# RamSaw/PipelineDP

Measured on AMD Instinct MI355X. Metric: records/sec DPEngine.aggregate COUNT+SUM at 1/2/4/8 MI355X; % HBM roofline, higher is better.
Workload: dtype f64; 1 GPU; configs[1]: 1e+09 records / 1e+07 privacy ids / 1e+06 Zipf(1.1) partitions per GPU, COUNT+SUM+PRIVACY_ID_COUNT, private partition selection; records_per_gpu=1000000000, privacy_ids_per_gpu=10000000, partitions=1000000, max_partitions_contributed=8, max_contributions_per_partition=2, noise=laplace, selection=truncated_geometric, parallelism=pid-sharded x1, privacy_id_range_supplied=True

## Files before the change

### pipelinedp_amd/csrc/dpg_api.hip

```cpp
#include <dlfcn.h>
#include <hip/hip_runtime.h>
#include <rccl/rccl.h>

#include <algorithm>
#include <cstddef>
#include <chrono>
#include <cmath>
#include <cstdio>
#include <cstdlib>
#include <cstring>
#include <map>
#include <mutex>
#include <string>
#include <thread>
#include <tuple>
#include <vector>

static hipError_t occ_query(int *blocks, const void *kern, int threads, size_t lds) {
    static std::mutex mu;
    static std::map<std::tuple<int, const void *, int, size_t>, int> cache;
    int dev = 0;
    (void)hipGetDevice(&dev);
    std::lock_guard<std::mutex> g(mu);
    const auto key = std::make_tuple(dev, kern, threads, lds);
// ... 29 lines not shown
#include "dpg_strkey.h"
#include "dpg_owner.h"
#include "dpg_pairx.h"
#include "dpg_partition.h"
#include "dpg_quantile.h"
#include "dpg_records.h"
#include "dpg_rsort.h"
#include "dpg_sample.h"
#include "dpg_select.h"
#include "dpg_shard.h"
#include "dpg_sortb.h"
#include "dpg_sortmw.h"
#include "dpg_team.h"
#include "dpg_utility.h"
#include "dpg_vsum.h"
#include "dpg_wave.h"
#include "dpg_hist_phases.h"

using namespace dpg;

namespace {

constexpr uint32_t kBucketTarget = 256;
constexpr uint32_t kMaxB1 = 11, kMaxB2 = 12, kMaxBR = 11;
constexpr uint32_t kMaxB1W = 12;
constexpr int kIptL1W = 8;
constexpr uint32_t kPinErr = 4096;
constexpr uint32_t kChunkGroup = 32;
constexpr int kRedoLevel2 = -100;
#ifndef DPG_PC_HALF
#define DPG_PC_HALF 0
#endif
#ifndef DPG_IPT_PC
#define DPG_IPT_PC 8
#endif

struct Buf {
    void *p = nullptr;
    size_t bytes = 0;
};

struct Control {
    uint32_t err;
    uint32_t item_cursor;
    uint32_t ntiles[8];
    int64_t n_scalar;
    uint32_t n_chunks;
    uint32_t n_over;
    uint32_t n_over2;
    uint32_t n_mchunks;
    uint32_t heavy_nfb;
    uint32_t pad_;
    uint32_t seg_paths[2];
    unsigned long long over_records;
    unsigned long long over2_records;
    unsigned long long pid_lo, pid_hi;
};

}

struct dpg_ctx {
    int device = 0;
    uint64_t seed = 0;
    int n_cu = 256;
    std::string err;
    std::map<std::string, Buf> bufs;
    std::vector<std::string> stage_names;
    std::vector<hipEvent_t> events;
    int n_events_used = 0;
    hipStream_t last_stream = nullptr;
    uint32_t bucket_target = 0;
    uint32_t bucket_cap = kBCap;
    void *comm = nullptr;
    const uint32_t *last_err = nullptr;
    int rank = 0, nranks = 1;
    char *stage_buf = nullptr;
    size_t stage_cap = 0, stage_head = 0;
    std::map<hipStream_t, hipEvent_t> stage_done;
    uint32_t *pin_tot = nullptr;
    hipEvent_t tot_ev = nullptr;
    uint32_t team_backoff = 0;
    uint32_t team_backoff_next = 64;
};

namespace {

int watchdog_seconds() {
#if defined(DPG_WATCHDOG) || defined(DPG_PHASE_TIMING)
    const char *e = std::getenv("DPG_WATCHDOG_S");
    return e ? std::atoi(e) : 0;
#else
    return 0;
#endif
}

uint32_t *watchdog_buffer(size_t n) {
    static uint32_t *buf = nullptr;
    static size_t cap = 0;
    if (n > cap) {
        if (buf) (void)hipHostFree(buf);
        if (hipHostMalloc((void **)&buf, n * 4, hipHostMallocCoherent) != hipSuccess) return nullptr;
        cap = n;
    }
    std::memset(buf, 0, n * 4);
    return buf;
}
// ... 1051 lines not shown
    WS(rbase, int64_t, "pieces.rbase", (size_t)8 * F);
    WS(cum, uint32_t, "pieces.cum", (size_t)8 * F);
    WS(tot, uint32_t, "pieces.tot", F);
    WS(ptot, uint32_t, "pieces.ptot", F);
    WS(ostart, int64_t, "pieces.ostart", F);
    WS(pdesc, PieceDesc, "pieces.desc", F);
    HIP_TRY(hipMemsetAsync(cum, 0, (size_t)8 * F * 4, s));
    HIP_TRY(hipMemsetAsync(&ctl->ntiles[0], 0, 4, s));
    stage(ctx, s, "partition1:pieces");
    k_region_base<<<(8 * F + 255) / 256, 256, 0, s>>>(rbase, F, C);
    LAUNCH_CHECK();
    k_build_tiles_single<<<(nt + 255) / 256, 256, 0, s>>>(n, sub, 1u, tiles, stb, snt,
                                                         &ctl->ntiles[0], XcdQueues{});
    LAUNCH_CHECK();
    using Src = SrcSoAKey<R, true>;
    constexpr size_t lds = scatter_lds<Src, R, IPT, FMAX, NT>();
    static_assert(lds <= (size_t)160 * 1024 * NT / kScatThreads - 512, "scatter LDS");
    if (F > (uint32_t)FMAX) return fail(ctx, DPG_ERR_HIP, "internal: piece level fan-out too large");
    auto kern = k_scatter<Src, R, IPT, FMAX, false, NT>;
    if (bits <= (uint32_t)agg_bits()) return fail(ctx, DPG_ERR_HIP, "internal: piece level fan-out");
    (void)set_func_attr((const void *)kern, hipFuncAttributeMaxDynamicSharedMemorySize,
                              (int)lds);
    const uint32_t gs = std::min<uint32_t>(nt, (uint32_t)ctx->n_cu * (kScatThreads / NT));
    if (int r = scat_phase_begin(ctx, s)) return r;
    kern<<<gs, NT, lds, s>>>(src, tiles, &ctl->ntiles[0], F, bits, nullptr, rbase, out,
                             XcdQueues{}, nullptr, nullptr, nullptr, 1u, cum, C,
                             (uint32_t)((uint64_t)8 * F * C), &ctl->err);
    LAUNCH_CHECK();
    if (int r = scat_phase_end(ctx, s, "partition1:pieces", gs)) return r;
    k_piece_totals<<<1, 1024, 0, s>>>(cum, rbase, F, tot, ptot, ostart, pdesc);
    LAUNCH_CHECK();
    if (!ctx->tot_ev && hipEventCreateWithFlags(&ctx->tot_ev, hipEventDisableTiming) != hipSuccess)
        return fail(ctx, DPG_ERR_HIP, "hipEventCreate (totals)");
    HIP_TRY(hipMemcpyAsync(host_tot, tot, (size_t)F * 4, hipMemcpyDeviceToHost, s));
    HIP_TRY(hipMemcpyAsync(host_tot + kPinErr, &ctl->err, 4, hipMemcpyDeviceToHost, s));
    HIP_TRY(hipEventRecord(ctx->tot_ev, s));
    *pt = PieceTab{rbase, cum, tot, ptot, ostart, F, pdesc};
    return DPG_OK;
}

template <class R>
int run_team_level2(dpg_ctx *ctx, hipStream_t s, const SrcAoS<R> &src, uint32_t S, uint32_t F2,
                    const int64_t *seg_start, const uint32_t *seg_cnt, R *out, Control *ctl,
                    int64_t **base_out, uint32_t **tot_out, const PieceTab *pt,
                    uint64_t max_bucket) {
    int st = DPG_OK;
    const uint32_t F = kTeamF;
    const size_t words = (size_t)8 * 3 * F + 8 * kTeamArriveStride + 32;
    WS(tw, uint32_t, "team.sync", words);
    WS(base, int64_t, "partition2.base", (size_t)S * F2);
    WS(tot, uint32_t, "partition2.tot", (size_t)S * F2);
    HIP_TRY(hipMemsetAsync(tw, 0, words * 4, s));
    uint32_t *abort_flag = tw + (size_t)8 * 3 * F + 8 * kTeamArriveStride;
    const TeamSync ts{tw, tw + (size_t)8 * 3 * F, abort_flag, &ctl->err};
    if (std::getenv("DPG_DEBUG_TEAM_ABORT")) {
        const uint32_t one = 1;
        UPLOAD(abort_flag, &one, 4);
        k_set_bits<<<1, 1, 0, s>>>(&ctl->err, 8u);
        LAUNCH_CHECK();
    }
    uint32_t sub_cap = (uint32_t)kTeamSub;
    if (const char *e = std::getenv("DPG_DEBUG_TEAM_SUB"))
        sub_cap = std::min<uint32_t>(sub_cap, std::max<uint32_t>(2, (uint32_t)std::atoi(e)) & ~1u);
    const uint32_t T = (uint32_t)ctx->n_cu / 8;
    const bool multi = (max_bucket + 8 + T - 1) / T + 2 > sub_cap;
    const void *k = pt ? (const void *)k_part2_team<R, true> : (const void *)k_part2_team<R, false>;
    (void)set_func_attr(k, hipFuncAttributeMaxDynamicSharedMemorySize, (int)team_lds<R>());
    stage(ctx, s, "partition2:team");
    if (pt)
        k_part2_team<R, true><<<(unsigned)ctx->n_cu, kScatThreads, team_lds<R>(), s>>>(
            src, seg_start, seg_cnt, S, F2, out, base, tot, ts, *pt, sub_cap);
    else
        k_part2_team<R, false><<<(unsigned)ctx->n_cu, kScatThreads, team_lds<R>(), s>>>(
            src, seg_start, seg_cnt, S, F2, out, base, tot, ts, PieceTab{}, sub_cap);
    LAUNCH_CHECK();
    if (multi) {
        stage(ctx, s, "partition2:team_multi");
        HIP_TRY(hipMemsetAsync(tw, 0, ((size_t)8 * 3 * F + 8 * kTeamArriveStride) * 4, s));
        const void *km = pt ? (const void *)k_part2_team<R, true, true>
                            : (const void *)k_part2_team<R, false, true>;
        (void)set_func_attr(km, hipFuncAttributeMaxDynamicSharedMemorySize, (int)team_lds<R>());
        if (pt)
            k_part2_team<R, true, true><<<(unsigned)ctx->n_cu, kScatThreads, team_lds<R>(), s>>>(
                src, seg_start, seg_cnt, S, F2, out, base, tot, ts, *pt, sub_cap);
        else
            k_part2_team<R, false, true><<<(unsigned)ctx->n_cu, kScatThreads, team_lds<R>(), s>>>(
                src, seg_start, seg_cnt, S, F2, out, base, tot, ts, PieceTab{}, sub_cap);
        LAUNCH_CHECK();
    }
    *base_out = base;
    *tot_out = tot;
    return DPG_OK;
}

template <class R>
int pipeline(dpg_ctx *ctx, hipStream_t s, const int64_t *pid, const int64_t *pk,
             const double *value, int64_t n, const dpg_bound_params *p, const dpg_partials *out,
             Control *ctl, const Plan &pl, int64_t pid_min, uint64_t U, uint32_t ib, PaOut *pa) {
    int st = DPG_OK;
    const bool var = (p->metric_mask & (DPG_M_MEAN | DPG_M_VARIANCE)) != 0;
    const Fmt f{ib, pl.pkbits, pl.kbits, pl.b1};
    const HashK H = make_hash(pl.kbits);
    const uint32_t F1 = 1u << pl.b1;
    SrcSoAKey<R> s1{pid, pk, p->public_mask, pl.P, pid_min, U, H, f,
                    low_mask(pl.kbits - pl.b1 + pl.pkbits), pl.kbits - pl.b1, &ctl->err};
    s1.value = value;
    int64_t *bstart = nullptr;
    uint32_t *bcnt = nullptr;
#ifndef DPG_L1_XCD
#define DPG_L1_XCD 0
#endif
#ifndef DPG_L1_SUBS
#define DPG_L1_SUBS 1
#endif
#ifndef DPG_L2_SUBS
#define DPG_L2_SUBS 1
#endif
    auto env_int = [](const char *name, int dflt) {
        const char *e = std::getenv(name);
        return e ? std::atoi(e) : dflt;
    };
    const bool l1_xcd = env_int("DPG_L1_XCD", DPG_L1_XCD) != 0;
    const int l1_subs = env_int("DPG_L1_SUBS", DPG_L1_SUBS);
    const int l2_subs = env_int("DPG_L2_SUBS", DPG_L2_SUBS);
#ifndef DPG_L1_GRP
#define DPG_L1_GRP 1
#endif
#ifndef DPG_L2_GRP
#define DPG_L2_GRP 1
#endif
    const bool l1_grp = env_int("DPG_L1_GRP", DPG_L1_GRP) != 0;
    const bool l2_grp = env_int("DPG_L2_GRP", DPG_L2_GRP) != 0;
    const uint32_t shift2 = pl.pkbits + (pl.kbits - pl.b1) - pl.b2;
    const uint32_t team_T = (uint32_t)ctx->n_cu / 8;
    const bool backoff = ctx->team_backoff > 0;
    if (backoff) {
        --ctx->team_backoff;
        stage(ctx, s, "team_backoff");
    }
    bool team = sizeof(R) == 8 && pl.b2 >= 6 && pl.b2 <= kMaxB1 && ctx->n_cu % 8 == 0 && team_T > 0 && l1_grp &&
                env_int("DPG_TEAM_L2", 1) != 0 && !backoff;
// ... 344 lines not shown
    if (!w) return nullptr;
    if (hipMemsetAsync(w, 0, 4, s) != hipSuccess) {
        *status = fail(ctx, DPG_ERR_HIP, "hipMemsetAsync (error word)");
        return nullptr;
    }
    ctx->last_err = w;
    return w;
}

}

extern "C" {

dpg_ctx *dpg_ctx_create(int device, uint64_t seed) {
    if (hipSetDevice(device) != hipSuccess) return nullptr;
    dpg_ctx *c = new dpg_ctx();
    c->device = device;
    c->seed = seed;
    hipDeviceProp_t prop;
    if (hipGetDeviceProperties(&prop, device) == hipSuccess) c->n_cu = prop.multiProcessorCount;
    return c;
}

void dpg_ctx_destroy(dpg_ctx *c) {
    if (!c) return;
    (void)hipSetDevice(c->device);
    if (c->comm && rccl().ok) (void)rccl().comm_destroy(static_cast<ncclComm_t>(c->comm));
    for (auto &kv : c->bufs)
        if (kv.second.p) (void)hipFree(kv.second.p);
    for (auto e : c->events) (void)hipEventDestroy(e);
    for (auto &kv : c->stage_done) {
        (void)hipEventSynchronize(kv.second);
        (void)hipEventDestroy(kv.second);
    }
    if (c->stage_buf) (void)hipHostFree(c->stage_buf);
    if (c->tot_ev) (void)hipEventDestroy(c->tot_ev);
    if (c->pin_tot) (void)hipHostFree(c->pin_tot);
    delete c;
}

int dpg_last_error(dpg_ctx *c, char *buf, size_t len) {
    if (!c || !buf || len == 0) return DPG_ERR_INVALID_ARG;
    std::snprintf(buf, len, "%s", c->err.c_str());
    return DPG_OK;
}

int dpg_set_seed(dpg_ctx *c, uint64_t seed) {
    if (!c) return DPG_ERR_INVALID_ARG;
    c->seed = seed;
    return DPG_OK;
}

uint64_t dpg_stream_seed(uint64_t seed, uint64_t nonce) { return stream_seed(seed, nonce); }

int dpg_set_tuning(dpg_ctx *ctx, int32_t bucket_target, int32_t bucket_cap) {
    if (!ctx) return DPG_ERR_INVALID_ARG;
    if (bucket_target > 0) ctx->bucket_target = (uint32_t)bucket_target;
    if (bucket_cap > 0) ctx->bucket_cap = std::min<uint32_t>((uint32_t)bucket_cap, kBCap);
    return DPG_OK;
}

int dpg_bound_aggregate(dpg_ctx *ctx, const int64_t *pid, const int64_t *pk, const double *value,
                        int64_t n, const dpg_bound_params *p, dpg_partials *out, void *stream) {
    if (!ctx) return DPG_ERR_INVALID_ARG;
    if (!p || !out || n < 0 || (n > 0 && (!pid || !pk)))
        return fail(ctx, DPG_ERR_INVALID_ARG, "null argument");
    if (p->n_partitions <= 0 || p->n_partitions >= 0xFFFFFFFFll)
        return fail(ctx, DPG_ERR_INVALID_ARG, "n_partitions must be in [1, 2^32-1)");
    if (out->n_partitions != p->n_partitions || !out->rows || !out->count)
        return fail(ctx, DPG_ERR_INVALID_ARG, "partials must cover n_partitions");
    if (p->mode < 0 || p->mode > 2) return fail(ctx, DPG_ERR_INVALID_ARG, "bad mode");
    const bool per_pid = p->mode == DPG_MODE_PER_PRIVACY_ID;
    if (per_pid ? p->max_contributions <= 0
                : (p->max_partitions_contributed <= 0 || p->max_contributions_per_partition <= 0))
        return fail(ctx, DPG_ERR_INVALID_ARG, "contribution bounds must be positive");
    if (n >= 0xFFFFFFFFll) return fail(ctx, DPG_ERR_UNSUPPORTED, "n must be < 2^32 per device");
    if (p->pid_count < 0 || p->pid_count > (1ll << 32))
        return fail(ctx, DPG_ERR_INVALID_ARG, "pid_count must be in [0, 2^32]");
    const bool var = (p->metric_mask & (DPG_M_MEAN | DPG_M_VARIANCE)) != 0;
    const bool need_values = (p->metric_mask & (DPG_M_SUM | DPG_M_MEAN | DPG_M_VARIANCE)) != 0;
    if (need_values && n > 0 && !value)
        return fail(ctx, DPG_ERR_INVALID_ARG, "value array required for SUM/MEAN/VARIANCE");
    if (var && out->nsum == nullptr)
        return fail(ctx, DPG_ERR_INVALID_ARG, "MEAN/VARIANCE need nsum/nsq partials");
    if (need_values && !var && out->sum == nullptr)
        return fail(ctx, DPG_ERR_INVALID_ARG, "SUM needs sum partials");
    (void)hipSetDevice(ctx->device);
    hipStream_t s = (hipStream_t)stream;
    ctx->stage_names.clear();
    ctx->n_events_used = 0;
    ctx->last_stream = s;
    int st = DPG_OK;
    const int64_t P = p->n_partitions;
    stage(ctx, s, "begin");
    HIP_TRY(hipMemsetAsync(out->rows, 0, P * 8, s));
    HIP_TRY(hipMemsetAsync(out->count, 0, P * 8, s));
    if (out->sum) HIP_TRY(hipMemsetAsync(out->sum, 0, P * 8, s));
    if (out->nsum) HIP_TRY(hipMemsetAsync(out->nsum, 0, P * 8, s));
    if (out->nsq) HIP_TRY(hipMemsetAsync(out->nsq, 0, P * 8, s));
    if (n == 0) return DPG_OK;
    return aggregate_impl(ctx, pid, pk, value, n, p, out, nullptr, s);
}

int dpg_preaggregate(dpg_ctx *ctx, const int64_t *pid, const int64_t *pk, const double *value,
                     int64_t n, const dpg_bound_params *p, dpg_pair_entry *pairs,
                     int64_t capacity, int64_t *partition_start, int64_t *n_pairs, void *stream) {
// ... 1600 lines not shown
```

### pipelinedp_amd/csrc/dpg_common.h

```cpp
#pragma once

#include <hip/hip_runtime.h>
#include <stdint.h>

#include "../../include/dpg.h"

#define DPG_WAVE 64

namespace dpg {

struct alignas(8) R8 {
    uint64_t w;
};
struct alignas(4) R12 {
    uint32_t lo, hi, idx;
};
struct alignas(16) R16 {
    uint64_t w;
    double v;
};

struct Fmt {
    uint32_t ib;
    uint32_t pkbits;
// ... 249 lines not shown
}

__device__ __forceinline__ double laplace_noise(double x, double b, const uint32_t u[4],
                                                const Gran &G) {
    if (!(b > 0)) return x;
    const double bg = b * G.ig;
    double e1 = -log(u53(u[0], u[1]));
    double e2 = -log(u53(u[2], u[3]));
    double k = floor(e1 * bg) - floor(e2 * bg);
    return rint(x * G.ig) * G.g + k * G.g;
}

__device__ __forceinline__ double gaussian_noise(double x, double sigma, const uint32_t u[4],
                                                 const Gran &G) {
    if (!(sigma > 0)) return x;
    double r = sqrt(-2.0 * log(u53(u[0], u[1])));
    double z = r * cos(6.283185307179586476925286766559 * u53(u[2], u[3]));
    return rint(x * G.ig) * G.g + rint(sigma * z * G.ig) * G.g;
}

__device__ __forceinline__ double add_noise(int kind, double x, double scale, const Gran &G,
                                            uint64_t seed, uint64_t pk, uint32_t slot) {
    if (kind == DPG_NOISE_NONE) return x;
    uint32_t c[4] = {(uint32_t)pk, (uint32_t)(pk >> 32), slot, 0u};
    philox4x32_10(c, (uint32_t)seed, (uint32_t)(seed >> 32) ^ DPG_TAG_NOISE);
    return kind == DPG_NOISE_GAUSSIAN ? gaussian_noise(x, scale, c, G)
                                      : laplace_noise(x, scale, c, G);
}

__device__ __forceinline__ void select_uniforms(uint64_t seed, uint64_t pk, uint32_t c[4]) {
    c[0] = (uint32_t)pk;
    c[1] = (uint32_t)(pk >> 32);
    c[2] = 0u;
    c[3] = 0u;
    philox4x32_10(c, (uint32_t)seed, (uint32_t)(seed >> 32) ^ DPG_TAG_SELECT);
}

__device__ __forceinline__ double clampd(double x, double lo, double hi) {
    return x < lo ? lo : (x > hi ? hi : x);
}

__device__ __forceinline__ uint32_t wave_excl_scan(uint32_t x, uint32_t &total) {
    int v = (int)x;
    v += __builtin_amdgcn_update_dpp(0, v, 0x111, 0xf, 0xf, true);
    v += __builtin_amdgcn_update_dpp(0, v, 0x112, 0xf, 0xf, true);
    v += __builtin_amdgcn_update_dpp(0, v, 0x114, 0xf, 0xf, true);
    v += __builtin_amdgcn_update_dpp(0, v, 0x118, 0xf, 0xf, true);
    v += __builtin_amdgcn_update_dpp(0, v, 0x142, 0xa, 0xf, false);
    v += __builtin_amdgcn_update_dpp(0, v, 0x143, 0xc, 0xf, false);
    total = (uint32_t)__builtin_amdgcn_readlane(v, 63);
    return (uint32_t)v - x;
}

}
```

### pipelinedp_amd/csrc/dpg_team.h

```cpp
#pragma once

#include "dpg_partition.h"

namespace dpg {

constexpr int kTeamIPT = 16;
#ifndef DPG_TEAM_PF
#define DPG_TEAM_PF 1
#endif
#ifndef DPG_TEAM_PF_PC
#define DPG_TEAM_PF_PC 1
#endif
#ifndef DPG_TEAM_WB
#define DPG_TEAM_WB 4
#endif
constexpr uint32_t kTeamF = 2048;
constexpr int kTeamSub = kScatThreads * kTeamIPT;
constexpr uint64_t kTeamTimeout = 50000000ull;
constexpr uint32_t kTeamArriveStride = 32;

struct TeamSync {
    uint32_t *tot;
    uint32_t *arrive;
    uint32_t *abort;
    uint32_t *err;
};

template <class R>
constexpr size_t team_lds() {
    return sizeof(R) * (kTeamSub + 1) + (size_t)kTeamF * 12 + 4 * 4 + 64;
}

__device__ __forceinline__ uint32_t ld_agent(const uint32_t *p) {
    return __hip_atomic_load(p, __ATOMIC_RELAXED, __HIP_MEMORY_SCOPE_AGENT);
}

struct NoOp {
    __device__ __forceinline__ void operator()() const {}
};
template <class F = NoOp>
__device__ __forceinline__ bool team_barrier(const TeamSync &ts, uint32_t team, uint32_t target,
                                             uint32_t *sh_ok, const F &between = F{}) {
    asm volatile("s_waitcnt vmcnt(0)" ::: "memory");
    __syncthreads();
    uint32_t *ctr = ts.arrive + team * kTeamArriveStride;
    uint32_t seen = 0;
    if (threadIdx.x == 0) {
        __hip_atomic_fetch_add(ctr, 1u, __ATOMIC_RELAXED, __HIP_MEMORY_SCOPE_AGENT);
        seen = ld_agent(ctr);
    }
    between();
    if (threadIdx.x == 0) {
        const uint64_t t0 = wall_clock64();
        uint32_t ok = 1;
        for (; seen < target; seen = ld_agent(ctr)) {
            if (ld_agent(ts.abort)) {
                ok = 0;
                break;
            }
            if (wall_clock64() - t0 > kTeamTimeout) {
                atomicOr(ts.abort, 1u);
                atomicOr(ts.err, 8u);
                ok = 0;
                break;
            }
            __builtin_amdgcn_s_sleep(2);
        }
        *sh_ok = ok;
    }
    __syncthreads();
    return *sh_ok != 0;
}

struct PieceDesc {
    uint32_t n;
    uint32_t pad0;
    int64_t ostart;
    int64_t base0;
    uint32_t ppre[8];
    uint32_t dl[8];
    uint32_t cend[8];
    uint32_t pad1[2];
};
static_assert(sizeof(PieceDesc) == 128, "PieceDesc is two 64-byte scalar loads");

struct PieceTab {
    const int64_t *rbase;
    const uint32_t *cum;
    const uint32_t *tot;
    const uint32_t *ptot;
    const int64_t *ostart;
    uint32_t F1;
    const PieceDesc *desc = nullptr;
};

typedef uint32_t u32x16 __attribute__((ext_vector_type(16)));
__device__ __forceinline__ void sload_desc(const PieceDesc *p, u32x16 &a, u32x16 &b) {
    p = uniform_ptr(p);
    asm volatile("s_load_dwordx16 %0, %2, 0x0\n\ts_load_dwordx16 %1, %2, 0x40\n\ts_waitcnt lgkmcnt(0)"
                 : "=s"(a), "=s"(b)
                 : "s"(p)
                 : "memory");
}

template <class R, bool kPc = false, bool kMulti = false>
__global__ __launch_bounds__(kScatThreads) void k_part2_team(SrcAoS<R> src,
                                                             const int64_t *seg_start,
                                                             const uint32_t *seg_cnt, uint32_t S,
                                                             uint32_t F2, R *out, int64_t *base_out,
                                                             uint32_t *tot_out, TeamSync ts,
                                                             PieceTab pt = PieceTab{},
                                                             uint32_t sub_cap = kTeamSub) {
    constexpr int IPT = kTeamIPT;
    constexpr int SUB = kTeamSub;
    constexpr uint32_t F = kTeamF;
    constexpr int DPT = F / kScatThreads;
    using W = Words<R>;
    extern __shared__ __attribute__((aligned(16))) char smem[];
    W *stage = reinterpret_cast<W *>(smem);
    uint32_t *cnt = reinterpret_cast<uint32_t *>(smem + sizeof(R) * (SUB + 1));
    uint32_t *dstart = cnt + F;
    uint32_t *cur = dstart + F + 1;
    uint32_t *sh16 = cur + F;
    __shared__ uint32_t sh_ok;
    const uint32_t team = blockIdx.x & 7u;
    const uint32_t T = gridDim.x >> 3;
    const uint32_t m = blockIdx.x >> 3;
    const int tid = threadIdx.x;
    const int lane = tid & 63, wv = tid >> 6;
    for (uint32_t d = tid; d < F; d += kScatThreads) cnt[d] = 0;
    __syncthreads();
    auto elem = [tid](int j) -> uint32_t {
        return (uint32_t)((j >> 1) * 2 * kScatThreads + 2 * tid + (j & 1));
    };
    auto share = [&](uint32_t s, int64_t &st, uint32_t &n, uint32_t &b0, uint32_t &lim) {
        n = __builtin_amdgcn_readfirstlane(kPc ? pt.ptot[s] : seg_cnt[s]);
        const int64_t st0 = kPc ? pt.ostart[s] : seg_start[s];
        st = (int64_t)(((uint64_t)__builtin_amdgcn_readfirstlane((uint32_t)((uint64_t)st0 >> 32)) << 32) |
                       (uint32_t)__builtin_amdgcn_readfirstlane((uint32_t)st0));
        const uint32_t q = kPc ? (((n + T - 1) / T + 1) & ~1u) : (n + T - 1) / T;
        b0 = min(n, m * q);
        lim = min(n, b0 + q) - b0;
    };
    R rec[IPT];
    uint32_t vmask = ~0u;
    auto load = [&](int64_t base, uint32_t lim) {
        if (lim >= 2) {
#pragma unroll
            for (int mm = 0; mm < IPT / 2; ++mm) {
                const uint32_t o = mm * 2 * kScatThreads + 2 * tid;
                const uint32_t a = min(o, lim - 2);
                R x0, x1;
                src.fetch2(base + a, x0, x1);
                rec[2 * mm] = a == o ? x0 : x1;
                rec[2 * mm + 1] = x1;
            }
        } else {
#pragma unroll
            for (int j = 0; j < IPT; ++j) rec[j] = lim ? src.fetch(base) : R{};
        }
    };
    auto load_pieces = [&](uint32_t s, uint32_t b0, uint32_t lim) {
        uint32_t ppre[8], dl[8], pc[8];
        const int64_t rb0 = pt.rbase[s];
        const int64_t base0 = (int64_t)(((uint64_t)__builtin_amdgcn_readfirstlane((uint32_t)((uint64_t)rb0 >> 32)) << 32) |
                                        (uint32_t)__builtin_amdgcn_readfirstlane((uint32_t)rb0));
        uint32_t acc = 0;
#pragma unroll
        for (int p = 0; p < 8; ++p) {
            const uint32_t off = __builtin_amdgcn_readfirstlane(
                (uint32_t)(pt.rbase[(size_t)p * pt.F1 + s] - rb0));
            pc[p] = __builtin_amdgcn_readfirstlane(pt.cum[(size_t)p * pt.F1 + s]);
            ppre[p] = acc;
            dl[p] = off - acc;
            acc += (pc[p] + 1u) & ~1u;
        }
        const char *bp = reinterpret_cast<const char *>(src.a + base0);
        uint32_t vm = 0;
#pragma unroll
        for (int mm = 0; mm < IPT / 2; ++mm) {
            const uint32_t o = mm * 2 * kScatThreads + 2 * tid;
            const uint32_t i = b0 + min(o, lim - 2);
            uint32_t d = dl[0], c = pc[0] + ppre[0];
#pragma unroll
            for (int p = 1; p < 8; ++p) {
                const bool in = i >= ppre[p];
                d = in ? dl[p] : d;
                c = in ? pc[p] + ppre[p] : c;
            }
            R x0, x1;
            const uint32_t boff = (i + d) * (uint32_t)sizeof(R);
            static_assert(sizeof(R) == 8, "piece-mode teams read 8-byte records");
            const u64x2 w = *reinterpret_cast<const u64x2 *>(bp + boff);
            const uint64_t w0 = w.x, w1 = w.y;
            __builtin_memcpy(&x0, &w0, sizeof(R));
            __builtin_memcpy(&x1, &w1, sizeof(R));
            rec[2 * mm] = x0;
            rec[2 * mm + 1] = x1;
            vm |= (i < c ? 1u : 0u) << (2 * mm);
            vm |= (i + 1 < c ? 1u : 0u) << (2 * mm + 1);
        }
        vmask = vm;
    };
    auto load_pieces_desc = [&](const u32x16 &da, const u32x16 &db, uint32_t b0, uint32_t lim) {
        const int64_t base0 = (int64_t)(((uint64_t)da[5] << 32) | da[4]);
        uint32_t ppre[8], dl[8], ce[8];
#pragma unroll
        for (int p = 0; p < 8; ++p) {
            ppre[p] = da[6 + p];
            dl[p] = p < 2 ? da[14 + p] : db[p - 2];
            ce[p] = db[6 + p];
        }
        const char *bp = reinterpret_cast<const char *>(src.a + base0);
        uint32_t vm = 0;
#pragma unroll
        for (int mm = 0; mm < IPT / 2; ++mm) {
            const uint32_t o = mm * 2 * kScatThreads + 2 * tid;
            const uint32_t i = b0 + min(o, lim - 2);
            uint32_t d = dl[0], c = ce[0];
#pragma unroll
            for (int p = 1; p < 8; ++p) {
                const bool in = i >= ppre[p];
                d = in ? dl[p] : d;
                c = in ? ce[p] : c;
            }
            R x0, x1;
            const uint32_t boff = (i + d) * (uint32_t)sizeof(R);
            const u64x2 w = *reinterpret_cast<const u64x2 *>(bp + boff);
            const uint64_t w0 = w.x, w1 = w.y;
            __builtin_memcpy(&x0, &w0, sizeof(R));
            __builtin_memcpy(&x1, &w1, sizeof(R));
            rec[2 * mm] = x0;
            rec[2 * mm + 1] = x1;
            vm |= (i < c ? 1u : 0u) << (2 * mm);
            vm |= (i + 1 < c ? 1u : 0u) << (2 * mm + 1);
        }
        vmask = vm;
    };
    uint32_t k = 0;
    constexpr bool kPF = DPG_TEAM_PF && (!kPc || DPG_TEAM_PF_PC) && !kMulti;
    auto share_q = [&](uint32_t n) -> uint32_t {
        return kPc ? (((n + T - 1) / T + 1) & ~1u) : (n + T - 1) / T;
    };
    auto next_nonempty = [&](uint32_t s) -> uint32_t {
        for (; s < S; s += 8) {
            const uint32_t n = __builtin_amdgcn_readfirstlane(kPc ? pt.ptot[s] : seg_cnt[s]);
            if (n != 0 && share_q(n) <= sub_cap) break;
        }
        return s;
    };
    int64_t pf_st = 0;
    uint32_t pf_n = 0, pf_b0 = 0, pf_lim = 0;
    constexpr bool use_desc = kPc && kPF;
    auto load_share = [&](uint32_t s) {
        if constexpr (kPc) {
            if constexpr (use_desc) {
                u32x16 da, db;
                sload_desc(pt.desc + min(s, S - 1), da, db);
                pf_n = __builtin_amdgcn_readfirstlane(da[0]);
                pf_st = (int64_t)(((uint64_t)da[3] << 32) | da[2]);
                const uint32_t q = ((pf_n + T - 1) / T + 1) & ~1u;
                pf_b0 = min(pf_n, m * q);
                pf_lim = min(pf_n, pf_b0 + q) - pf_b0;
                load_pieces_desc(da, db, pf_b0, max(pf_lim, 2u));
                return;
            }
        }
        share(s, pf_st, pf_n, pf_b0, pf_lim);
        if constexpr (kPc) {
            vmask = 0;
            if (pf_lim > 0) load_pieces(s, pf_b0, pf_lim);
        } else {
            load(pf_st + pf_b0, pf_lim);
        }
    };
    uint32_t pf_s = S;
    if constexpr (kPF) {
        pf_s = next_nonempty(team);
        if (use_desc || pf_s < S) load_share(pf_s);
    }
    auto write_out = [&](int64_t st, uint32_t nv) {
        constexpr int WB = DPG_TEAM_WB;
        for (uint32_t k0 = 0; k0 < nv; k0 += WB * kScatThreads) {
            W x[WB];
            uint32_t dd[WB], kc[WB];
#pragma unroll
            for (int u = 0; u < WB; ++u) {
                kc[u] = min(k0 + u * kScatThreads + tid, nv - 1);
                x[u] = stage[kc[u]];
                dd[u] = src.digit(from_words<R>(x[u]));
            }
            uint32_t c1[WB], c2[WB];
#pragma unroll
            for (int u = 0; u < WB; ++u) {
                c1[u] = cur[dd[u]];
                c2[u] = dstart[dd[u]];
            }
#pragma unroll
            for (int u = 0; u < WB; ++u)
                *reinterpret_cast<W *>(&out[st + c1[u] + (kc[u] - c2[u])]) = x[u];
        }
    };
    for (uint32_t s = team; s < S; s += 8) {
        int64_t st;
        uint32_t n, b0, lim;
        if constexpr (kPF) {
            if (s == pf_s) {
                st = pf_st;
                n = pf_n;
                b0 = pf_b0;
                lim = pf_lim;
            } else {
                share(s, st, n, b0, lim);
            }
        } else {
            share(s, st, n, b0, lim);
        }
        if constexpr (kMulti) {
            if (n == 0 || share_q(n) <= sub_cap) continue;
        } else {
            if (n == 0) {
                if (m == 0)
                    for (uint32_t d = tid; d < F2; d += kScatThreads) {
                        base_out[(size_t)s * F2 + d] = st;
                        tot_out[(size_t)s * F2 + d] = 0;
                    }
                continue;
            }
            if (share_q(n) > sub_cap) continue;
        }
        auto team_starts = [&](const uint32_t *tt) {
            const uint32_t d0 = DPT * tid;
            uint32_t c[DPT], x = 0;
#pragma unroll
            for (int u = 0; u < DPT; ++u) {
                c[u] = ld_agent(&tt[d0 + u]);
                x += c[u];
            }
            uint32_t wt;
            uint32_t e = wave_excl_scan(x, wt);
            if (lane == 63) sh16[wv] = wt;
            __syncthreads();
#pragma unroll
            for (int w = 0; w < kScatThreads / 64; ++w)
                if (w < wv) e += sh16[w];
            uint32_t *tz = ts.tot + ((size_t)team * 3 + (k + 1) % 3) * F;
#pragma unroll
            for (int u = 0; u < DPT; ++u) {
                cur[d0 + u] += e;
                if (m == 0) {
                    if (d0 + u < F2) {
                        base_out[(size_t)s * F2 + d0 + u] = st + e;
                        tot_out[(size_t)s * F2 + d0 + u] = c[u];
                    }
                    __hip_atomic_store(&tz[d0 + u], 0u, __ATOMIC_RELAXED, __HIP_MEMORY_SCOPE_AGENT);
                }
                e += c[u];
            }
        };
        if constexpr (kMulti) {
            const uint32_t q = share_q(n);
            {
                uint32_t *tt = ts.tot + ((size_t)team * 3 + k % 3) * F;
                const uint32_t J = (q + sub_cap - 1) / sub_cap;
                auto load_part = [&](uint32_t j, uint32_t &lj) {
                    const uint32_t bj = b0 + j * sub_cap;
                    lj = lim > j * sub_cap ? min(sub_cap, lim - j * sub_cap) : 0u;
                    if constexpr (kPc) {
                        if constexpr (use_desc) {
                            u32x16 da, db;
                            sload_desc(pt.desc + s, da, db);
                            load_pieces_desc(da, db, bj, max(lj, 2u));
                        } else {
                            vmask = 0;
                            if (lj > 0) load_pieces(s, bj, lj);
                        }
                    } else {
                        load(st + bj, lj);
                    }
                };
                auto ok_elem = [&](int jj, uint32_t lj) {
                    bool ok = elem(jj) < lj;
                    if constexpr (kPc) ok = ok && ((vmask >> jj) & 1u);
                    return ok;
                };
                for (uint32_t j = 0; j < J; ++j) {
                    uint32_t lj;
                    load_part(j, lj);
#pragma unroll
                    for (int jj = 0; jj < IPT; ++jj) {
                        const bool ok = ok_elem(jj, lj);
                        atomicAdd(&cnt[ok ? src.digit(rec[jj]) : 0u], ok ? 1u : 0u);
                    }
                }
                __syncthreads();
                {
                    const uint32_t d0 = DPT * tid;
#pragma unroll
                    for (int u = 0; u < DPT; ++u) {
                        cur[d0 + u] = atomicAdd(&tt[d0 + u], cnt[d0 + u]);
                        cnt[d0 + u] = 0;
                    }
                }
                ++k;
                if (!team_barrier(ts, team, T * k, &sh_ok)) return;
                team_starts(tt);
                for (uint32_t j = 0; j < J; ++j) {
                    __syncthreads();
                    uint32_t lj;
                    load_part(j, lj);
                    uint32_t drm[IPT];
#pragma unroll
                    for (int jj = 0; jj < IPT; ++jj) {
                        const bool ok = ok_elem(jj, lj);
                        const uint32_t dg = ok ? src.digit(rec[jj]) : 0u;
                        const uint32_t rk = atomicAdd(&cnt[dg], ok ? 1u : 0u);
                        drm[jj] = ok ? (dg | (rk << 12)) : ~0u;
                    }
                    __syncthreads();
                    const uint32_t d0 = DPT * tid;
                    uint32_t c[DPT], x = 0;
#pragma unroll
                    for (int u = 0; u < DPT; ++u) {
                        c[u] = cnt[d0 + u];
                        x += c[u];
                    }
                    uint32_t wt;
                    uint32_t e = wave_excl_scan(x, wt);
                    if (lane == 63) sh16[wv] = wt;
                    __syncthreads();
                    uint32_t nvj = 0;
#pragma unroll
                    for (int w = 0; w < kScatThreads / 64; ++w) {
                        if (w < wv) e += sh16[w];
                        nvj += sh16[w];
                    }
#pragma unroll
                    for (int u = 0; u < DPT; ++u) {
                        dstart[d0 + u] = e;
                        cnt[d0 + u] = 0;
                        e += c[u];
                    }
                    __syncthreads();
#pragma unroll
                    for (int jj = 0; jj < IPT; ++jj) {
                        const uint32_t pos = drm[jj] != ~0u ? dstart[drm[jj] & 0xFFFu] + (drm[jj] >> 12)
                                                            : (uint32_t)SUB;
                        stage[pos] = to_words(rec[jj]);
                    }
                    __syncthreads();
                    write_out(st, nvj);
                    __syncthreads();
#pragma unroll
                    for (int u = 0; u < DPT; ++u) cur[d0 + u] += c[u];
                }
                __syncthreads();
                continue;
            }
        } else {
        uint32_t *tt = ts.tot + ((size_t)team * 3 + k % 3) * F;
        if constexpr (!kPF) load_share(s);
        uint32_t dr[IPT];
        uint32_t nv = 0;
        {
            uint32_t dg[IPT];
            bool okv[IPT];
#pragma unroll
            for (int j = 0; j < IPT; ++j) {
                okv[j] = elem(j) < lim;
                if constexpr (kPc) okv[j] = okv[j] && ((vmask >> j) & 1u);
                dg[j] = okv[j] ? src.digit(rec[j]) : 0u;
            }
            uint32_t rk[IPT];
#pragma unroll
            for (int j = 0; j < IPT; ++j) rk[j] = atomicAdd(&cnt[dg[j]], okv[j] ? 1u : 0u);
#pragma unroll
            for (int j = 0; j < IPT; ++j) dr[j] = okv[j] ? (dg[j] | (rk[j] << 12)) : ~0u;
        }
        __syncthreads();
        {
            const uint32_t d0 = DPT * tid;
            uint32_t c[DPT], x = 0;
#pragma unroll
            for (int u = 0; u < DPT; ++u) {
                c[u] = cnt[d0 + u];
                x += c[u];
            }
            uint32_t o[DPT];
#pragma unroll
            for (int u = 0; u < DPT; ++u) o[u] = atomicAdd(&tt[d0 + u], c[u]);
            uint32_t wt;
            uint32_t e = wave_excl_scan(x, wt);
            if (lane == 63) sh16[wv] = wt;
            __syncthreads();
#pragma unroll
            for (int w = 0; w < kScatThreads / 64; ++w) {
                if (w < wv) e += sh16[w];
                nv += sh16[w];
            }
#pragma unroll
            for (int u = 0; u < DPT; ++u) {
                dstart[d0 + u] = e;
                if constexpr (!kPF) cur[d0 + u] = o[u];
                cnt[d0 + u] = 0;
                e += c[u];
            }
            if (tid == 0) dstart[F] = nv;
            if constexpr (kPF) {
                __syncthreads();
#pragma unroll
                for (int j = 0; j < IPT; ++j) {
                    const uint32_t pos = dr[j] != ~0u ? dstart[dr[j] & 0xFFFu] + (dr[j] >> 12) : (uint32_t)SUB;
                    stage[pos] = to_words(rec[j]);
                }
#pragma unroll
                for (int u = 0; u < DPT; ++u) cur[d0 + u] = o[u];
                pf_s = next_nonempty(s + 8);
            }
        }
        ++k;
        auto prefetch = [&]() {
            if constexpr (kPF) {
                if (use_desc || pf_s < S) load_share(pf_s);
            }
        };
        if (!team_barrier(ts, team, T * k, &sh_ok, prefetch)) return;
        {
            const uint32_t d0 = DPT * tid;
            uint32_t c[DPT], x = 0;
#pragma unroll
            for (int u = 0; u < DPT; ++u) {
                c[u] = ld_agent(&tt[d0 + u]);
                x += c[u];
            }
            uint32_t wt;
            uint32_t e = wave_excl_scan(x, wt);
            if (lane == 63) sh16[wv] = wt;
            __syncthreads();
#pragma unroll
            for (int w = 0; w < kScatThreads / 64; ++w)
                if (w < wv) e += sh16[w];
            uint32_t *tz = ts.tot + ((size_t)team * 3 + (k + 1) % 3) * F;
#pragma unroll
            for (int u = 0; u < DPT; ++u) {
                cur[d0 + u] += e;
                if (m == 0) {
                    if (d0 + u < F2) {
                        base_out[(size_t)s * F2 + d0 + u] = st + e;
                        tot_out[(size_t)s * F2 + d0 + u] = c[u];
                    }
                    __hip_atomic_store(&tz[d0 + u], 0u, __ATOMIC_RELAXED, __HIP_MEMORY_SCOPE_AGENT);
                }
                e += c[u];
            }
        }
        if constexpr (!kPF) {
#pragma unroll
            for (int j = 0; j < IPT; ++j) {
                const uint32_t pos = dr[j] != ~0u ? dstart[dr[j] & 0xFFFu] + (dr[j] >> 12) : (uint32_t)SUB;
                stage[pos] = to_words(rec[j]);
            }
        }
        __syncthreads();
        {
            constexpr int WB = DPG_TEAM_WB;
            for (uint32_t k0 = 0; k0 < nv; k0 += WB * kScatThreads) {
                W x[WB];
                uint32_t dd[WB], kc[WB];
#pragma unroll
                for (int u = 0; u < WB; ++u) {
                    kc[u] = min(k0 + u * kScatThreads + tid, nv - 1);
                    x[u] = stage[kc[u]];
                    dd[u] = src.digit(from_words<R>(x[u]));
                }
                uint32_t c1[WB], c2[WB];
#pragma unroll
                for (int u = 0; u < WB; ++u) {
                    c1[u] = cur[dd[u]];
                    c2[u] = dstart[dd[u]];
                }
#pragma unroll
                for (int u = 0; u < WB; ++u)
                    *reinterpret_cast<W *>(&out[st + c1[u] + (kc[u] - c2[u])]) = x[u];
            }
        }
        __syncthreads();
        }
    }
}

}
```

Measured before the change: 56.81 billion records/s.

## Resolve team piece spans once per share and use DPP block prefix scan

In piece-descriptor mode, each share's descriptor is now resolved once on scalar registers into at most two pieces, so per-item address calculation becomes a single compare instead of an 8-way select chain. The full lookup path is kept as a fallback and reloads the descriptor when a share spans more than two pieces. The cross-wave prefix over the 16 per-wave totals now uses DPP lane shifts and readlane instead of a serial loop. It also adds an optional, default-off descriptor lookahead and debug path counters, at the cost of extra code and higher scalar register pressure.

```diff
diff --git a/pipelinedp_amd/csrc/dpg_api.hip b/pipelinedp_amd/csrc/dpg_api.hip
--- a/pipelinedp_amd/csrc/dpg_api.hip
+++ b/pipelinedp_amd/csrc/dpg_api.hip
@@ -105,6 +105,7 @@
     uint32_t heavy_nfb;
     uint32_t pad_;
     uint32_t seg_paths[2];
+    uint32_t team_paths[2];
     unsigned long long over_records;
     unsigned long long over2_records;
     unsigned long long pid_lo, pid_hi;
@@ -1262,7 +1263,9 @@
     WS(tot, uint32_t, "partition2.tot", (size_t)S * F2);
     HIP_TRY(hipMemsetAsync(tw, 0, words * 4, s));
     uint32_t *abort_flag = tw + (size_t)8 * 3 * F + 8 * kTeamArriveStride;
-    const TeamSync ts{tw, tw + (size_t)8 * 3 * F, abort_flag, &ctl->err};
+    TeamSync ts{tw, tw + (size_t)8 * 3 * F, abort_flag, &ctl->err};
+    const bool dbg_paths = pt && std::getenv("DPG_DEBUG_TEAM_PATHS");
+    if (dbg_paths) ts.paths = ctl->team_paths;
     if (std::getenv("DPG_DEBUG_TEAM_ABORT")) {
         const uint32_t one = 1;
         UPLOAD(abort_flag, &one, 4);
@@ -1297,6 +1300,13 @@
             k_part2_team<R, false, true><<<(unsigned)ctx->n_cu, kScatThreads, team_lds<R>(), s>>>(
                 src, seg_start, seg_cnt, S, F2, out, base, tot, ts, PieceTab{}, sub_cap);
         LAUNCH_CHECK();
+    }
+    if (dbg_paths) {
+        uint32_t hp[2];
+        HIP_TRY(hipMemcpyAsync(hp, ctl->team_paths, sizeof(hp), hipMemcpyDeviceToHost, s));
+        HIP_TRY(hipStreamSynchronize(s));
+        if (hp[0]) stage(ctx, s, "team.pieces=pair");
+        if (hp[1]) stage(ctx, s, "team.pieces=lookup");
     }
     *base_out = base;
     *tot_out = tot;
@@ -1747,6 +1757,23 @@
 }
 
 uint64_t dpg_stream_seed(uint64_t seed, uint64_t nonce) { return stream_seed(seed, nonce); }
+
+void dpg_debug_team_resolve(const uint32_t *ppre, const uint32_t *dl, const uint32_t *ce, uint32_t b0,
+                            uint32_t lim, uint32_t *out) {
+    uint32_t a[8], b[8], c[8];
+    for (int p = 0; p < 8; ++p) {
+        a[p] = ppre[p];
+        b[p] = dl[p];
+        c[p] = ce[p];
+    }
+    const dpg::PieceSpan r = dpg::team_resolve(a, b, c, b0, lim);
+    out[0] = r.bnd;
+    out[1] = r.dl0;
+    out[2] = r.ce0;
+    out[3] = r.dl1;
+    out[4] = r.ce1;
+    out[5] = r.pair;
+}
 
 int dpg_set_tuning(dpg_ctx *ctx, int32_t bucket_target, int32_t bucket_cap) {
     if (!ctx) return DPG_ERR_INVALID_ARG;
diff --git a/pipelinedp_amd/csrc/dpg_common.h b/pipelinedp_amd/csrc/dpg_common.h
--- a/pipelinedp_amd/csrc/dpg_common.h
+++ b/pipelinedp_amd/csrc/dpg_common.h
@@ -325,4 +325,16 @@
     return (uint32_t)v - x;
 }
 
-}
+__device__ __forceinline__ uint32_t block_prefix16(const uint32_t *sh16, uint32_t &total) {
+    const uint32_t w = __builtin_amdgcn_readfirstlane(threadIdx.x >> 6);
+    int v = (int)sh16[threadIdx.x & 15u];
+    v += __builtin_amdgcn_update_dpp(0, v, 0x111, 0xf, 0xf, true);
+    v += __builtin_amdgcn_update_dpp(0, v, 0x112, 0xf, 0xf, true);
+    v += __builtin_amdgcn_update_dpp(0, v, 0x114, 0xf, 0xf, true);
+    v += __builtin_amdgcn_update_dpp(0, v, 0x118, 0xf, 0xf, true);
+    total = (uint32_t)__builtin_amdgcn_readlane(v, 15);
+    const uint32_t below = (uint32_t)__builtin_amdgcn_readlane(v, (int)(w ? w - 1u : 0u));
+    return w ? below : 0u;
+}
+
+}
diff --git a/pipelinedp_amd/csrc/dpg_team.h b/pipelinedp_amd/csrc/dpg_team.h
--- a/pipelinedp_amd/csrc/dpg_team.h
+++ b/pipelinedp_amd/csrc/dpg_team.h
@@ -13,6 +13,15 @@
 #endif
 #ifndef DPG_TEAM_WB
 #define DPG_TEAM_WB 4
+#endif
+#ifndef DPG_TEAM_PAIR
+#define DPG_TEAM_PAIR 1
+#endif
+#ifndef DPG_TEAM_DESC_AHEAD
+#define DPG_TEAM_DESC_AHEAD 0
+#endif
+#ifndef DPG_TEAM_SCAN1
+#define DPG_TEAM_SCAN1 1
 #endif
 constexpr uint32_t kTeamF = 2048;
 constexpr int kTeamSub = kScatThreads * kTeamIPT;
@@ -24,6 +33,7 @@
     uint32_t *arrive;
     uint32_t *abort;
     uint32_t *err;
+    uint32_t *paths = nullptr;
 };
 
 template <class R>
@@ -101,6 +111,104 @@
                  : "=s"(a), "=s"(b)
                  : "s"(p)
                  : "memory");
+}
+__device__ __forceinline__ void sload_desc_early(const PieceDesc *p, u32x16 &a, u32x16 &b) {
+    typedef const u32x16 __attribute__((address_space(4))) * ConstVec;
+    const ConstVec q = (ConstVec)(uintptr_t)uniform_ptr(p);
+    a = q[0];
+    b = q[1];
+}
+
+struct PieceSpan {
+    uint32_t bnd, dl0, ce0, dl1, ce1, pair;
+};
+__host__ __device__ inline PieceSpan team_resolve(const uint32_t (&ppre)[8], const uint32_t (&dl)[8],
+                                                  const uint32_t (&ce)[8], uint32_t b0, uint32_t lim) {
+    const uint32_t i0 = b0, i1 = b0 + (lim > 2u ? lim : 2u) - 2u;
+    PieceSpan r{ppre[0], dl[0], ce[0], dl[0], ce[0], 0u};
+    const uint32_t n0 = ~i0, n1 = ~i1;
+    uint32_t m0[8], m1[8];
+#pragma unroll
+    for (int p = 1; p < 8; ++p) {
+        m0[p] = (uint32_t)((int32_t)(ppre[p] + n0) >> 31);
+        m1[p] = (uint32_t)((int32_t)(ppre[p] + n1) >> 31);
+#ifdef __HIP_DEVICE_COMPILE__
+        asm("" : "+s"(m0[p]), "+s"(m1[p]));
+#endif
+        r.dl0 ^= (r.dl0 ^ dl[p]) & m0[p];
+        r.ce0 ^= (r.ce0 ^ ce[p]) & m0[p];
+        r.dl1 ^= (r.dl1 ^ dl[p]) & m1[p];
+        r.ce1 ^= (r.ce1 ^ ce[p]) & m1[p];
+        r.bnd ^= (r.bnd ^ ppre[p]) & m1[p];
+    }
+    uint32_t mid = 0;
+#pragma unroll
+    for (int p = 1; p < 7; ++p)
+        mid |= ~m0[p] & m1[p + 1] & (uint32_t)((int32_t)(ppre[p] - ppre[p + 1]) >> 31);
+    r.pair = ~mid & 1u;
+    return r;
+}
+
+__device__ __forceinline__ uint32_t team_addr_lookup(const u32x16 &da, const u32x16 &db, uint32_t b0,
+                                                     uint32_t lim, uint32_t (&boff)[kTeamIPT / 2]) {
+    uint32_t ppre[8], dl[8], ce[8];
+#pragma unroll
+    for (int p = 0; p < 8; ++p) {
+        ppre[p] = da[6 + p];
+        dl[p] = p < 2 ? da[14 + p] : db[p - 2];
+        ce[p] = db[6 + p];
+    }
+    uint32_t vm = 0;
+#pragma unroll
+    for (int mm = 0; mm < kTeamIPT / 2; ++mm) {
+        const uint32_t o = mm * 2 * kScatThreads + 2 * threadIdx.x;
+        const uint32_t i = b0 + min(o, lim - 2);
+        uint32_t d = dl[0], c = ce[0];
+#pragma unroll
+        for (int p = 1; p < 8; ++p) {
+            const bool in = i >= ppre[p];
+            d = in ? dl[p] : d;
+            c = in ? ce[p] : c;
+        }
+        boff[mm] = (i + d) * 8u;
+        vm |= (i < c ? 1u : 0u) << (2 * mm);
+        vm |= (i + 1 < c ? 1u : 0u) << (2 * mm + 1);
+    }
+    return vm;
+}
+__device__ __forceinline__ uint32_t team_addr_pair(const PieceSpan &sp, uint32_t b0, uint32_t lim,
+                                                   uint32_t (&boff)[kTeamIPT / 2]) {
+    uint32_t vm = 0;
+#pragma unroll
+    for (int mm = 0; mm < kTeamIPT / 2; ++mm) {
+        const uint32_t o = mm * 2 * kScatThreads + 2 * threadIdx.x;
+        const uint32_t i = b0 + min(o, lim - 2);
+        const bool in = i >= sp.bnd;
+        const uint32_t d = in ? sp.dl1 : sp.dl0, c = in ? sp.ce1 : sp.ce0;
+        boff[mm] = (i + d) * 8u;
+        vm |= (i < c ? 1u : 0u) << (2 * mm);
+        vm |= (i + 1 < c ? 1u : 0u) << (2 * mm + 1);
+    }
+    return vm;
+}
+template <class R>
+__device__ __forceinline__ void team_fetch(const R *a, int64_t base0, uint32_t (&boff)[kTeamIPT / 2],
+                                           uint32_t &vm, R (&rec)[kTeamIPT]) {
+    static_assert(sizeof(R) == 8 && kTeamIPT == 16, "piece-mode teams read 8-byte records");
+    asm volatile(""
+                 : "+v"(boff[0]), "+v"(boff[1]), "+v"(boff[2]), "+v"(boff[3]), "+v"(boff[4]),
+                   "+v"(boff[5]), "+v"(boff[6]), "+v"(boff[7]), "+v"(vm));
+    const char *bp = reinterpret_cast<const char *>(a + base0);
+#pragma unroll
+    for (int mm = 0; mm < kTeamIPT / 2; ++mm) {
+        R x0, x1;
+        const u64x2 w = *reinterpret_cast<const u64x2 *>(bp + boff[mm]);
+        const uint64_t w0 = w.x, w1 = w.y;
+        __builtin_memcpy(&x0, &w0, sizeof(R));
+        __builtin_memcpy(&x1, &w1, sizeof(R));
+        rec[2 * mm] = x0;
+        rec[2 * mm + 1] = x1;
+    }
 }
 
 template <class R, bool kPc = false, bool kMulti = false>
@@ -203,38 +311,23 @@
         vmask = vm;
     };
     auto load_pieces_desc = [&](const u32x16 &da, const u32x16 &db, uint32_t b0, uint32_t lim) {
-        const int64_t base0 = (int64_t)(((uint64_t)da[5] << 32) | da[4]);
-        uint32_t ppre[8], dl[8], ce[8];
-#pragma unroll
-        for (int p = 0; p < 8; ++p) {
-            ppre[p] = da[6 + p];
-            dl[p] = p < 2 ? da[14 + p] : db[p - 2];
-            ce[p] = db[6 + p];
-        }
-        const char *bp = reinterpret_cast<const char *>(src.a + base0);
-        uint32_t vm = 0;
-#pragma unroll
-        for (int mm = 0; mm < IPT / 2; ++mm) {
-            const uint32_t o = mm * 2 * kScatThreads + 2 * tid;
-            const uint32_t i = b0 + min(o, lim - 2);
-            uint32_t d = dl[0], c = ce[0];
-#pragma unroll
-            for (int p = 1; p < 8; ++p) {
-                const bool in = i >= ppre[p];
-                d = in ? dl[p] : d;
-                c = in ? ce[p] : c;
-            }
-            R x0, x1;
-            const uint32_t boff = (i + d) * (uint32_t)sizeof(R);
-            const u64x2 w = *reinterpret_cast<const u64x2 *>(bp + boff);
-            const uint64_t w0 = w.x, w1 = w.y;
-            __builtin_memcpy(&x0, &w0, sizeof(R));
-            __builtin_memcpy(&x1, &w1, sizeof(R));
-            rec[2 * mm] = x0;
-            rec[2 * mm + 1] = x1;
-            vm |= (i < c ? 1u : 0u) << (2 * mm);
-            vm |= (i + 1 < c ? 1u : 0u) << (2 * mm + 1);
-        }
+        uint32_t boff[IPT / 2];
+        uint32_t vm = team_addr_lookup(da, db, b0, lim, boff);
+        team_fetch<R>(src.a, (int64_t)(((uint64_t)da[5] << 32) | da[4]), boff, vm, rec);
+        vmask = vm;
+    };
+    auto load_span = [&](const PieceSpan &sp, int64_t base0, const PieceDesc *dp, uint32_t b0,
+                         uint32_t lim) {
+        uint32_t boff[IPT / 2];
+        uint32_t vm;
+        if (sp.pair) {
+            vm = team_addr_pair(sp, b0, lim, boff);
+        } else {
+            u32x16 da, db;
+            sload_desc(dp, da, db);
+            vm = team_addr_lookup(da, db, b0, lim, boff);
+        }
+        team_fetch<R>(src.a, base0, boff, vm, rec);
         vmask = vm;
     };
     uint32_t k = 0;
@@ -252,17 +345,54 @@
     int64_t pf_st = 0;
     uint32_t pf_n = 0, pf_b0 = 0, pf_lim = 0;
     constexpr bool use_desc = kPc && kPF;
+    constexpr bool kPair = use_desc && DPG_TEAM_PAIR;
+    constexpr bool kAhead = use_desc && DPG_TEAM_DESC_AHEAD;
+    PieceSpan pf_sp{};
+    int64_t pf_base0 = 0;
+    u32x16 pf_da = {}, pf_db = {};
+    uint32_t n_pair = 0, n_lookup = 0;
+    auto take_desc = [&](const u32x16 &da, const u32x16 &db) {
+        pf_n = __builtin_amdgcn_readfirstlane(da[0]);
+        pf_st = (int64_t)(((uint64_t)da[3] << 32) | da[2]);
+        const uint32_t q = ((pf_n + T - 1) / T + 1) & ~1u;
+        pf_b0 = min(pf_n, m * q);
+        pf_lim = min(pf_n, pf_b0 + q) - pf_b0;
+        if constexpr (kPair) {
+            uint32_t ppre[8], dl[8], ce[8];
+#pragma unroll
+            for (int p = 0; p < 8; ++p) {
+                ppre[p] = da[6 + p];
+                dl[p] = p < 2 ? da[14 + p] : db[p - 2];
+                ce[p] = db[6 + p];
+            }
+            pf_base0 = (int64_t)(((uint64_t)da[5] << 32) | da[4]);
+            pf_sp = team_resolve(ppre, dl, ce, pf_b0, pf_lim);
+            asm volatile(""
+                         : "+s"(pf_sp.bnd), "+s"(pf_sp.dl0), "+s"(pf_sp.ce0), "+s"(pf_sp.dl1),
+                           "+s"(pf_sp.ce1), "+s"(pf_sp.pair), "+s"(pf_b0), "+s"(pf_lim), "+s"(pf_base0));
+        } else {
+            pf_da = da;
+            pf_db = db;
+        }
+    };
+    auto issue_share = [&](uint32_t s) {
+        if constexpr (kPair) {
+            if (s < S) {
+                n_pair += pf_sp.pair;
+                n_lookup += 1u - pf_sp.pair;
+            }
+            load_span(pf_sp, pf_base0, pt.desc + min(s, S - 1), pf_b0, max(pf_lim, 2u));
+        } else {
+            load_pieces_desc(pf_da, pf_db, pf_b0, max(pf_lim, 2u));
+        }
+    };
     auto load_share = [&](uint32_t s) {
         if constexpr (kPc) {
             if constexpr (use_desc) {
                 u32x16 da, db;
                 sload_desc(pt.desc + min(s, S - 1), da, db);
-                pf_n = __builtin_amdgcn_readfirstlane(da[0]);
-                pf_st = (int64_t)(((uint64_t)da[3] << 32) | da[2]);
-                const uint32_t q = ((pf_n + T - 1) / T + 1) & ~1u;
-                pf_b0 = min(pf_n, m * q);
-                pf_lim = min(pf_n, pf_b0 + q) - pf_b0;
-                load_pieces_desc(da, db, pf_b0, max(pf_lim, 2u));
+                take_desc(da, db);
+                issue_share(s);
                 return;
             }
         }
@@ -341,9 +471,14 @@
             uint32_t e = wave_excl_scan(x, wt);
             if (lane == 63) sh16[wv] = wt;
             __syncthreads();
+#if DPG_TEAM_SCAN1
+            uint32_t all;
+            e += block_prefix16(sh16, all);
+#else
 #pragma unroll
             for (int w = 0; w < kScatThreads / 64; ++w)
                 if (w < wv) e += sh16[w];
+#endif
             uint32_t *tz = ts.tot + ((size_t)team * 3 + (k + 1) % 3) * F;
 #pragma unroll
             for (int u = 0; u < DPT; ++u) {
@@ -430,11 +565,15 @@
                     if (lane == 63) sh16[wv] = wt;
                     __syncthreads();
                     uint32_t nvj = 0;
+#if DPG_TEAM_SCAN1
+                    e += block_prefix16(sh16, nvj);
+#else
 #pragma unroll
                     for (int w = 0; w < kScatThreads / 64; ++w) {
                         if (w < wv) e += sh16[w];
                         nvj += sh16[w];
                     }
+#endif
 #pragma unroll
                     for (int u = 0; u < DPT; ++u) {
                         dstart[d0 + u] = e;
@@ -460,6 +599,8 @@
         } else {
         uint32_t *tt = ts.tot + ((size_t)team * 3 + k % 3) * F;
         if constexpr (!kPF) load_share(s);
+        u32x16 nda = {}, ndb = {};
+        if constexpr (kAhead) sload_desc_early(pt.desc + min(s + 8, S - 1), nda, ndb);
         uint32_t dr[IPT];
         uint32_t nv = 0;
         {
@@ -489,15 +630,32 @@
             uint32_t o[DPT];
 #pragma unroll
             for (int u = 0; u < DPT; ++u) o[u] = atomicAdd(&tt[d0 + u], c[u]);
+            if constexpr (kAhead) {
+                uint32_t ns = s + 8;
+                const uint32_t nn = __builtin_amdgcn_readfirstlane(nda[0]);
+                if (ns < S && (nn == 0 || share_q(nn) > sub_cap)) {
+                    ns = next_nonempty(ns + 8);
+                    u32x16 da, db;
+                    sload_desc(pt.desc + min(ns, S - 1), da, db);
+                    take_desc(da, db);
+                } else {
+                    take_desc(nda, ndb);
+                }
+                pf_s = ns;
+            }
             uint32_t wt;
             uint32_t e = wave_excl_scan(x, wt);
             if (lane == 63) sh16[wv] = wt;
             __syncthreads();
+#if DPG_TEAM_SCAN1
+            e += block_prefix16(sh16, nv);
+#else
 #pragma unroll
             for (int w = 0; w < kScatThreads / 64; ++w) {
                 if (w < wv) e += sh16[w];
                 nv += sh16[w];
             }
+#endif
 #pragma unroll
             for (int u = 0; u < DPT; ++u) {
                 dstart[d0 + u] = e;
@@ -515,12 +673,14 @@
                 }
 #pragma unroll
                 for (int u = 0; u < DPT; ++u) cur[d0 + u] = o[u];
-                pf_s = next_nonempty(s + 8);
+                if constexpr (!kAhead) pf_s = next_nonempty(s + 8);
             }
         }
         ++k;
         auto prefetch = [&]() {
-            if constexpr (kPF) {
+            if constexpr (kAhead) {
+                issue_share(pf_s);
+            } else if constexpr (kPF) {
                 if (use_desc || pf_s < S) load_share(pf_s);
             }
         };
@@ -537,9 +697,14 @@
             uint32_t e = wave_excl_scan(x, wt);
             if (lane == 63) sh16[wv] = wt;
             __syncthreads();
+#if DPG_TEAM_SCAN1
+            uint32_t all;
+            e += block_prefix16(sh16, all);
+#else
 #pragma unroll
             for (int w = 0; w < kScatThreads / 64; ++w)
                 if (w < wv) e += sh16[w];
+#endif
             uint32_t *tz = ts.tot + ((size_t)team * 3 + (k + 1) % 3) * F;
 #pragma unroll
             for (int u = 0; u < DPT; ++u) {
@@ -587,6 +752,12 @@
         __syncthreads();
         }
     }
-}
-
-}
+    if constexpr (kPair) {
+        if (ts.paths && tid == 0) {
+            atomicAdd(&ts.paths[0], n_pair);
+            atomicAdd(&ts.paths[1], n_lookup);
+        }
+    }
+}
+
+}
```

Measured after the change: 58.21 billion records/s, median of 6. 2.5% higher.
